# microsoft/VidTok

Measured on NVIDIA H100. Metric: frames/sec encode+decode, kl_causal_488 17x256x256, higher is better.
Workload: dtype bf16

## Files before the change

### vidtok_b200/csrc/tblock_tc.cu

```cuda
#include <cuda.h>

#include <cstdio>
#include <cstdlib>
#include <cstring>
#include <string>

#include "common.cuh"
#include "kernels.h"
#include "tc_ptx.cuh"

namespace vt {

namespace {
using namespace tcx;

thread_local std::string g_tb_err;
constexpr int kC = 128;
constexpr int kKc = kC / 64;
constexpr uint32_t kTile = 128 * 128;
constexpr int kHSlots = 3;
constexpr int kConsumerWarps = 8;
constexpr int kProducerWarp = kConsumerWarps;
constexpr int kThreadsTb = (kConsumerWarps + 4) * 32;

struct TbParams {
  int B, T, H, W;
  int BW, BH;
  int tilesW, tilesH;
  long long num_strips;
  int stages;
  const float* bias1;
  const float* bias2;
  const float* g2;
  const float* b2;
  int ln_out, ln_out_silu;
  const float* g3;
  const float* b3;
  const bf16* x;
  bf16* out;
  bf16* out2;
  const bf16* n1;
  int cached_in;
  const bf16* cn1_in;
  const bf16* ch_in;
  bf16* cn1_out;
  bf16* ch_out;
};
struct TbMaps {
  CUtensorMap n1, w1, w2, cn1;
};

__device__ __forceinline__ float quad_sum(float v) {
  v += __shfl_xor_sync(0xffffffffu, v, 1);
  v += __shfl_xor_sync(0xffffffffu, v, 2);
  return v;
}

template <bool kCache>
__global__ void __launch_bounds__(kThreadsTb, 1) tblock_tc_kernel(const __grid_constant__ TbMaps maps, const TbParams p) {
  extern __shared__ uint8_t smem_raw[];
  const uint32_t smem_base = (smem_u32(smem_raw) + 1023u) & ~1023u;
  uint8_t* smem_gen = smem_raw + (smem_base - smem_u32(smem_raw));
  const int warp = threadIdx.x >> 5, lane = threadIdx.x & 31;
  const uint32_t h_base = smem_base;
  const uint32_t ring_base = h_base + kHSlots * kKc * kTile;
  const uint32_t stage_bytes = 2u * kTile;
  const uint32_t bar_base = ring_base + (uint32_t)p.stages * stage_bytes;
  auto full_bar = [&](int s) { return bar_base + 8u * s; };
  auto empty_bar = [&](int s) { return bar_base + 8u * (p.stages + s); };
  float* cst = reinterpret_cast<float*>(smem_gen + (bar_base - smem_base) + 16u * p.stages);

  for (int i = threadIdx.x; i < kC; i += kThreadsTb) {
    cst[i] = p.bias1 ? p.bias1[i] : 0.f;
    cst[kC + i] = 0.5f * p.g2[i];
    cst[2 * kC + i] = 0.5f * p.b2[i];
    cst[3 * kC + i] = p.bias2 ? p.bias2[i] : 0.f;
    const float sc = p.ln_out_silu ? 0.5f : 1.0f;
    cst[4 * kC + i] = p.ln_out ? sc * p.g3[i] : 0.f;
    cst[5 * kC + i] = p.ln_out ? sc * p.b3[i] : 0.f;
  }
  if (threadIdx.x == 0) {
    for (int s = 0; s < p.stages; ++s) { mbar_init(full_bar(s), 1); mbar_init(empty_bar(s), kConsumerWarps); }
    asm volatile("fence.mbarrier_init.release.cluster;" ::: "memory");
  }
  __syncthreads();

  if (warp >= kProducerWarp) {
    asm volatile("setmaxnreg.dec.sync.aligned.u32 40;" ::: "memory");
    if (warp != kProducerWarp) return;
    const bool el = elect_one();
    if (el) { prefetch_tmap(&maps.n1); prefetch_tmap(&maps.w1); prefetch_tmap(&maps.w2); }
    const bool front = kCache && p.cached_in;
    int stage = 0;
    uint32_t phase = 0;
    auto acquire = [&](uint32_t bytes) {
      mbar_wait(empty_bar(stage), phase ^ 1u);
      if (el) mbar_expect_tx(full_bar(stage), bytes);
    };
    auto advance = [&]() { if (++stage == p.stages) { stage = 0; phase ^= 1u; } };
    for (long long strip = blockIdx.x; strip < p.num_strips; strip += gridDim.x) {
      const int tw = (int)(strip % p.tilesW);
      const int th = (int)((strip / p.tilesW) % p.tilesH);
      const int b = (int)(strip / ((long long)p.tilesW * p.tilesH));
      const int w0 = tw * p.BW, h0 = th * p.BH;
      for (int t = 0; t < p.T; ++t) {
        for (int a = 0; a < 3; ++a) {
          const int tv = t - 2 + a;
          if (tv < 0 && !front) continue;
          for (int kc = 0; kc < kKc; ++kc) {
            acquire(2u * kTile);
            if (el) {
              const uint32_t sa = ring_base + stage * stage_bytes;
              if (kCache && tv < 0) tma_load_5d(sa, &maps.cn1, full_bar(stage), kc * 64, w0, h0, tv + 2, b);
              else tma_load_5d(sa, &maps.n1, full_bar(stage), kc * 64, w0, h0, tv, b);
              tma_load_3d(sa + kTile, &maps.w1, full_bar(stage), a * kC + kc * 64, 0, 0);
            }
            advance();
          }
        }
        for (int a = 0; a < 3; ++a) {
          if (t - 2 + a < 0 && !front) continue;
          for (int kc = 0; kc < kKc; ++kc) {
            acquire(kTile);
            if (el) tma_load_3d(ring_base + stage * stage_bytes + kTile, &maps.w2, full_bar(stage), a * kC + kc * 64, 0, 0);
            advance();
          }
        }
      }
    }
    return;
  }

  asm volatile("setmaxnreg.inc.sync.aligned.u32 232;" ::: "memory");
  const int g = warp >> 2, wq = warp & 3;
  const uint32_t hi = desc_hi(1024u);
  float acc[kC / 2];
  int stage = 0, pend_stage = -1;
  uint32_t phase = 0;
  auto release = [&]() {
    if (lane == 0 && pend_stage >= 0) mbar_arrive(empty_bar(pend_stage));
    pend_stage = -1;
  };
  auto kstep = [&](bool a_from_stage, uint32_t h_addr, uint32_t scale) {
    mbar_wait(full_bar(stage), phase);
    const uint32_t sa = ring_base + stage * stage_bytes;
    const uint32_t al = desc_lo(a_from_stage ? sa + (uint32_t)g * 64u * 128u : h_addr), bl = desc_lo(sa + kTile);
    wgmma_fence();
#pragma unroll
    for (uint32_t j = 0; j < 4u; ++j) wgmma_k16<kC, false>(acc, desc(al + 2u * j, hi), desc(bl + 2u * j, hi), j == 0 ? scale : 1u);
    wgmma_commit();
    wgmma_wait<1>();
    release();
    pend_stage = stage;
    if (++stage == p.stages) { stage = 0; phase ^= 1u; }
  };
  auto finish = [&]() {
    wgmma_wait<0>();
    acc_fence(acc);
    release();
  };
  auto wg_sync = [&]() { asm volatile("bar.sync %0, 128;" ::"r"(1 + g) : "memory"); };
  const float* bias1 = cst;
  const float* g2 = cst + kC;
  const float* b2 = cst + 2 * kC;
  const float* bias2 = cst + 3 * kC;
  const float* g3 = cst + 4 * kC;
  const float* b3 = cst + 5 * kC;
  const int cq = 2 * (lane & 3);
  const int rbase = 64 * g + 16 * wq + (lane >> 2);
  const bool front = kCache && p.cached_in;
  const int gtid = threadIdx.x & 127;
  auto slot_of = [&](int tv) { return h_base + (uint32_t)((tv + kHSlots) % kHSlots) * kKc * kTile; };
  auto ring_unit = [&](uint32_t slot, int row, int c) {
    return reinterpret_cast<uint4*>(smem_gen + (slot - smem_base) + (c >> 6) * kTile + row * 128 + ((((c & 63) >> 3) ^ (row & 7)) << 4));
  };

  for (long long strip = blockIdx.x; strip < p.num_strips; strip += gridDim.x) {
    const int tw = (int)(strip % p.tilesW);
    const int th = (int)((strip / p.tilesW) % p.tilesH);
    const int b = (int)(strip / ((long long)p.tilesW * p.tilesH));
    long long pos0[2];
#pragma unroll
    for (int r = 0; r < 2; ++r) {
      const int row = rbase + 8 * r;
      const int h = th * p.BH + row / p.BW, w = tw * p.BW + row % p.BW;
      pos0[r] = (((long long)b * p.T) * p.H + h) * p.W + w;
    }
    const long long frame = (long long)p.H * p.W;
    auto cache_pos = [&](int i, int j, int& row) {
      row = 64 * g + (i >> 4);
      const int h = th * p.BH + row / p.BW, w = tw * p.BW + row % p.BW;
      return ((((long long)b * 2 + j) * p.H + h) * p.W + w) * kC + (i & 15) * 8;
    };
    if (front) {
      wg_sync();
      for (int j = 0; j < 2; ++j)
        for (int i = gtid; i < 64 * 16; i += 128) {
          int row;
          const long long off = cache_pos(i, j, row);
          *ring_unit(slot_of(j - 2), row, (i & 15) * 8) = *reinterpret_cast<const uint4*>(p.ch_in + off);
        }
      fence_async_smem();
      wg_sync();
    }
    for (int t = 0; t < p.T; ++t) {
      uint32_t scale = 0;
      for (int a = 0; a < 3; ++a) {
        if (t - 2 + a < 0 && !front) continue;
        for (int kc = 0; kc < kKc; ++kc) { kstep(true, 0u, scale); scale = 1; }
      }
      finish();
      wg_sync();
      const uint32_t slot = h_base + (uint32_t)(t % kHSlots) * kKc * kTile;
#pragma unroll
      for (int r = 0; r < 2; ++r) {
        float s = 0.f, q = 0.f;
#pragma unroll
        for (int j = 0; j < kC / 8; ++j) {
          const int c = 8 * j + cq;
          const float f0 = acc[4 * j + 2 * r] + bias1[c], f1 = acc[4 * j + 2 * r + 1] + bias1[c + 1];
          s += f0 + f1;
          q = fmaf(f0, f0, q);
          q = fmaf(f1, f1, q);
          const uint32_t kp = pack_bf16x2(f0, f1);
          acc[4 * j + 2 * r] = bf16_lo(kp);
          acc[4 * j + 2 * r + 1] = bf16_hi(kp);
        }
        const float mean = quad_sum(s) * (1.0f / kC);
        float var = fmaf(-mean, mean, quad_sum(q) * (1.0f / kC));
        var = var < 0.f ? 0.f : var;
        const float rstd = rsqrtf(var + 1e-6f);
        const float nmr = -mean * rstd;
        const int row = rbase + 8 * r;
        uint8_t* hrow = smem_gen + (slot - smem_base) + row * 128;
#pragma unroll
        for (int j = 0; j < kC / 8; ++j) {
          const int c = 8 * j + cq;
          float y0 = fmaf(fmaf(acc[4 * j + 2 * r], rstd, nmr), g2[c], b2[c]);
          float y1 = fmaf(fmaf(acc[4 * j + 2 * r + 1], rstd, nmr), g2[c + 1], b2[c + 1]);
          y0 = fmaf(y0, tanh_approx(y0), y0);
          y1 = fmaf(y1, tanh_approx(y1), y1);
          const int cc = c & 63, u = cc >> 3;
          *reinterpret_cast<uint32_t*>(hrow + (c >> 6) * kTile + ((u ^ (row & 7)) << 4) + (cc & 7) * 2) = pack_bf16x2(y0, y1);
        }
      }
      fence_async_smem();
      wg_sync();
      scale = 0;
      for (int a = 0; a < 3; ++a) {
        const int tv = t - 2 + a;
        if (tv < 0 && !front) continue;
        const uint32_t hs = (kCache ? slot_of(tv) : h_base + (uint32_t)(tv % kHSlots) * kKc * kTile) + (uint32_t)g * 64u * 128u;
        for (int kc = 0; kc < kKc; ++kc) { kstep(false, hs + (uint32_t)kc * kTile, scale); scale = 1; }
      }
      finish();
#pragma unroll
      for (int r = 0; r < 2; ++r) {
        const long long off = (pos0[r] + (long long)t * frame) * kC;
        const bf16* xr = p.x + off;
        bf16* orow = p.out + off;
        float s = 0.f, q = 0.f;
#pragma unroll
        for (int j = 0; j < kC / 8; ++j) {
          const int c = 8 * j + cq;
          const uint32_t xw = *reinterpret_cast<const uint32_t*>(xr + c);
          const float f0 = acc[4 * j + 2 * r] + bias2[c] + bf16_lo(xw), f1 = acc[4 * j + 2 * r + 1] + bias2[c + 1] + bf16_hi(xw);
          s += f0 + f1;
          q = fmaf(f0, f0, q);
          q = fmaf(f1, f1, q);
          const uint32_t kp = pack_bf16x2(f0, f1);
          *reinterpret_cast<uint32_t*>(orow + c) = kp;
          acc[4 * j + 2 * r] = bf16_lo(kp);
          acc[4 * j + 2 * r + 1] = bf16_hi(kp);
        }
        if (!p.ln_out) continue;
        const float mean = quad_sum(s) * (1.0f / kC);
        float var = fmaf(-mean, mean, quad_sum(q) * (1.0f / kC));
        var = var < 0.f ? 0.f : var;
        const float rstd = rsqrtf(var + 1e-6f);
        const float nmr = -mean * rstd;
        bf16* o2 = p.out2 + off;
#pragma unroll
        for (int j = 0; j < kC / 8; ++j) {
          const int c = 8 * j + cq;
          float y0 = fmaf(fmaf(acc[4 * j + 2 * r], rstd, nmr), g3[c], b3[c]);
          float y1 = fmaf(fmaf(acc[4 * j + 2 * r + 1], rstd, nmr), g3[c + 1], b3[c + 1]);
          if (p.ln_out_silu) {
            y0 = fmaf(y0, tanh_approx(y0), y0);
            y1 = fmaf(y1, tanh_approx(y1), y1);
          }
          *reinterpret_cast<uint32_t*>(o2 + c) = pack_bf16x2(y0, y1);
        }
      }
    }
    if (kCache) {
      for (int j = 0; j < 2; ++j) {
        const int tv = p.T - 2 + j;
        for (int i = gtid; i < 64 * 16; i += 128) {
          int row;
          const long long off = cache_pos(i, j, row);
          const long long pix = off - (((long long)b * 2 + j) * frame) * kC;
          uint4 hv = make_uint4(0u, 0u, 0u, 0u), nv = hv;
          if (tv >= 0 || front) hv = *ring_unit(slot_of(tv), row, (i & 15) * 8);
          if (tv >= 0) nv = *reinterpret_cast<const uint4*>(p.n1 + (((long long)b * p.T + tv) * frame) * kC + pix);
          else if (front) nv = *reinterpret_cast<const uint4*>(p.cn1_in + (((long long)b * 2 + tv + 2) * frame) * kC + pix);
          *reinterpret_cast<uint4*>(p.ch_out + off) = hv;
          *reinterpret_cast<uint4*>(p.cn1_out + off) = nv;
        }
      }
    }
  }
}

typedef CUresult (*EncodeTiledFn)(CUtensorMap*, CUtensorMapDataType, cuuint32_t, void*, const cuuint64_t*,
                                  const cuuint64_t*, const cuuint32_t*, const cuuint32_t*, CUtensorMapInterleave,
                                  CUtensorMapSwizzle, CUtensorMapL2promotion, CUtensorMapFloatOOBfill);
EncodeTiledFn tb_get_encode() {
  static EncodeTiledFn fn = nullptr;
  static bool tried = false;
  if (!tried) {
    tried = true;
    void* f = nullptr;
    cudaDriverEntryPointQueryResult q;
    if (cudaGetDriverEntryPoint("cuTensorMapEncodeTiled", &f, cudaEnableDefault, &q) == cudaSuccess && q == cudaDriverEntryPointSuccess)
      fn = (EncodeTiledFn)f;
  }
  return fn;
}

bool strip_box(int H, int W, int& BW, int& BH) {
  for (int bw = 128; bw >= 1; bw >>= 1) {
    if (W % bw != 0) continue;
    const int bh = 128 / bw;
    if (bh <= 256 && H % bh == 0) { BW = bw; BH = bh; return true; }
  }
  return false;
}
}

const char* tblock_tc_last_error() { return g_tb_err.c_str(); }

bool tblock_tc_supported(int B, int T, int H, int W, int C, bool planning) {
// ... 3 lines not shown
  if (!env) { g_tb_err = "disabled (VT_TBLOCK=0)"; return false; }
  if (C != kC) { g_tb_err = "C != 128"; return false; }
  if (B <= 0 || T <= 0) { g_tb_err = "empty"; return false; }
  int BW, BH;
  if (!strip_box(H, W, BW, BH)) { g_tb_err = "H x W not tileable by a 128-position box"; return false; }
  if (!planning && !tb_get_encode()) { g_tb_err = "cuTensorMapEncodeTiled unavailable"; return false; }
  return true;
}

cudaError_t launch_tblock_tc(const bf16* n1, const bf16* x, const bf16* w1, const float* bias1, const float* gamma2,
                             const float* beta2, const bf16* w2, const float* bias2, bf16* out, bf16* out2,
                             const float* gamma_out, const float* beta_out, bool out_silu, int B, int T, int H, int W,
                             cudaStream_t s, const TbCache* cache) {
  g_tb_err.clear();
  EncodeTiledFn enc = tb_get_encode();
  if (!enc) { g_tb_err = "cuTensorMapEncodeTiled unavailable"; return cudaErrorNotSupported; }
  TbParams p;
  memset(&p, 0, sizeof(p));
  if (!strip_box(H, W, p.BW, p.BH)) { g_tb_err = "H x W not tileable"; return cudaErrorInvalidValue; }
  p.B = B; p.T = T; p.H = H; p.W = W;
  p.tilesW = W / p.BW; p.tilesH = H / p.BH;
  p.num_strips = (long long)B * p.tilesH * p.tilesW;
  p.bias1 = bias1; p.bias2 = bias2; p.g2 = gamma2; p.b2 = beta2;
  p.ln_out = (out2 && gamma_out && beta_out) ? 1 : 0;
  p.ln_out_silu = out_silu ? 1 : 0;
  p.g3 = gamma_out; p.b3 = beta_out;
  p.x = x; p.out = out; p.out2 = out2;
  if (cache) {
    if (!cache->n1_out || !cache->h_out || (!cache->n1_in != !cache->h_in)) { g_tb_err = "cache: both outputs, and both or no inputs"; return cudaErrorInvalidValue; }
    p.n1 = n1;
    p.cached_in = cache->n1_in ? 1 : 0;
    p.cn1_in = cache->n1_in; p.ch_in = cache->h_in; p.cn1_out = cache->n1_out; p.ch_out = cache->h_out;
  }
  const size_t fixed = 1024 + (size_t)kHSlots * kKc * kTile + 6 * kC * 4;
  const size_t budget = 225 * 1024;
  int stages = (int)((budget - fixed) / (2 * kTile + 16));
  if (stages > 4) stages = 4;
  p.stages = stages;
  const size_t smem = fixed + (size_t)stages * (2 * kTile + 16);
  TbMaps maps;
  {
    cuuint64_t dims[5] = {(cuuint64_t)kC, (cuuint64_t)W, (cuuint64_t)H, (cuuint64_t)T, (cuuint64_t)B};
    cuuint64_t strides[4] = {(cuuint64_t)kC * 2, (cuuint64_t)W * kC * 2, (cuuint64_t)H * W * kC * 2, (cuuint64_t)T * H * W * kC * 2};
    cuuint32_t box[5] = {64, (cuuint32_t)p.BW, (cuuint32_t)p.BH, 1, 1};
    cuuint32_t es[5] = {1, 1, 1, 1, 1};
    CUresult r = enc(&maps.n1, CU_TENSOR_MAP_DATA_TYPE_BFLOAT16, 5, const_cast<bf16*>(n1), dims, strides, box, es, CU_TENSOR_MAP_INTERLEAVE_NONE,
                     CU_TENSOR_MAP_SWIZZLE_128B, CU_TENSOR_MAP_L2_PROMOTION_L2_256B, CU_TENSOR_MAP_FLOAT_OOB_FILL_NONE);
    if (r != CUDA_SUCCESS) { g_tb_err = "cuTensorMapEncodeTiled(n1) failed: " + std::to_string((int)r); return cudaErrorInvalidValue; }
    maps.cn1 = maps.n1;
    if (p.cached_in) {
      dims[3] = 2;
      strides[3] = 2ull * H * W * kC * 2;
      r = enc(&maps.cn1, CU_TENSOR_MAP_DATA_TYPE_BFLOAT16, 5, const_cast<bf16*>(p.cn1_in), dims, strides, box, es, CU_TENSOR_MAP_INTERLEAVE_NONE,
              CU_TENSOR_MAP_SWIZZLE_128B, CU_TENSOR_MAP_L2_PROMOTION_L2_256B, CU_TENSOR_MAP_FLOAT_OOB_FILL_NONE);
      if (r != CUDA_SUCCESS) { g_tb_err = "cuTensorMapEncodeTiled(n1 cache) failed: " + std::to_string((int)r); return cudaErrorInvalidValue; }
    }
  }
  for (int i = 0; i < 2; ++i) {
    cuuint64_t dims[3] = {(cuuint64_t)(3 * kC), (cuuint64_t)kC, 1};
    cuuint64_t strides[2] = {(cuuint64_t)(3 * kC) * 2, (cuuint64_t)(3 * kC) * kC * 2};
    cuuint32_t box[3] = {64, (cuuint32_t)kC, 1};
    cuuint32_t es[3] = {1, 1, 1};
    CUresult r = enc(i ? &maps.w2 : &maps.w1, CU_TENSOR_MAP_DATA_TYPE_BFLOAT16, 3, const_cast<bf16*>(i ? w2 : w1), dims, strides, box, es,
                     CU_TENSOR_MAP_INTERLEAVE_NONE, CU_TENSOR_MAP_SWIZZLE_128B, CU_TENSOR_MAP_L2_PROMOTION_L2_256B,
                     CU_TENSOR_MAP_FLOAT_OOB_FILL_NONE);
    if (r != CUDA_SUCCESS) { g_tb_err = "cuTensorMapEncodeTiled(weights) failed: " + std::to_string((int)r); return cudaErrorInvalidValue; }
  }
  static bool attr[64] = {false};
  static int sms[64] = {0};
  int dev = 0;
  cudaGetDevice(&dev);
  if (dev < 0 || dev >= 64) return cudaErrorInvalidDevice;
// ... 23 lines not shown
```

Before: 435.9.

## Process two frames per step so each weight tile feeds two WGMMA accumulators

Restructures the fused temporal block kernel to handle frame pairs. Each weight tile loaded through TMA is now reused for two output frames with two accumulator sets. The ring becomes single-tile slots (weights and activations loaded separately), and the h ring grows to four slots so both frames' history fits. The aim is to halve weight-tile traffic and barrier round trips per frame. Epilogue constants move from shared memory to __ldg reads, and an L2 prefetch of the residual input is added. The cost is doubled accumulator registers, which raises spill risk under the 232-register cap, and fewer effective pipeline stages.

```diff
diff --git a/vidtok_b200/csrc/tblock_tc.cu b/vidtok_b200/csrc/tblock_tc.cu
--- a/vidtok_b200/csrc/tblock_tc.cu
+++ b/vidtok_b200/csrc/tblock_tc.cu
@@ -4,6 +4,7 @@
 #include <cstdlib>
 #include <cstring>
 #include <string>
+#include <type_traits>
 
 #include "common.cuh"
 #include "kernels.h"
@@ -18,7 +19,8 @@
 constexpr int kC = 128;
 constexpr int kKc = kC / 64;
 constexpr uint32_t kTile = 128 * 128;
-constexpr int kHSlots = 3;
+constexpr int kHSlots = 4;
+constexpr int kTiles = 6;
 constexpr int kConsumerWarps = 8;
 constexpr int kProducerWarp = kConsumerWarps;
 constexpr int kThreadsTb = (kConsumerWarps + 4) * 32;
@@ -28,7 +30,6 @@
   int BW, BH;
   int tilesW, tilesH;
   long long num_strips;
-  int stages;
   const float* bias1;
   const float* bias2;
   const float* g2;
@@ -55,6 +56,12 @@
   v += __shfl_xor_sync(0xffffffffu, v, 2);
   return v;
 }
+template <typename T>
+__device__ __forceinline__ const T* opaque(const T* p) {
+  asm volatile("" : "+l"(p));
+  return p;
+}
+__device__ __forceinline__ void prefetch_l2(const void* p) { asm volatile("prefetch.global.L2 [%0];" ::"l"(p)); }
 
 template <bool kCache>
 __global__ void __launch_bounds__(kThreadsTb, 1) tblock_tc_kernel(const __grid_constant__ TbMaps maps, const TbParams p) {
@@ -64,68 +71,64 @@
   const int warp = threadIdx.x >> 5, lane = threadIdx.x & 31;
   const uint32_t h_base = smem_base;
   const uint32_t ring_base = h_base + kHSlots * kKc * kTile;
-  const uint32_t stage_bytes = 2u * kTile;
-  const uint32_t bar_base = ring_base + (uint32_t)p.stages * stage_bytes;
+  const uint32_t bar_base = ring_base + kTiles * kTile;
   auto full_bar = [&](int s) { return bar_base + 8u * s; };
-  auto empty_bar = [&](int s) { return bar_base + 8u * (p.stages + s); };
-  float* cst = reinterpret_cast<float*>(smem_gen + (bar_base - smem_base) + 16u * p.stages);
-
-  for (int i = threadIdx.x; i < kC; i += kThreadsTb) {
-    cst[i] = p.bias1 ? p.bias1[i] : 0.f;
-    cst[kC + i] = 0.5f * p.g2[i];
-    cst[2 * kC + i] = 0.5f * p.b2[i];
-    cst[3 * kC + i] = p.bias2 ? p.bias2[i] : 0.f;
-    const float sc = p.ln_out_silu ? 0.5f : 1.0f;
-    cst[4 * kC + i] = p.ln_out ? sc * p.g3[i] : 0.f;
-    cst[5 * kC + i] = p.ln_out ? sc * p.b3[i] : 0.f;
-  }
+  auto empty_bar = [&](int s) { return bar_base + 8u * (kTiles + s); };
   if (threadIdx.x == 0) {
-    for (int s = 0; s < p.stages; ++s) { mbar_init(full_bar(s), 1); mbar_init(empty_bar(s), kConsumerWarps); }
+    for (int s = 0; s < kTiles; ++s) { mbar_init(full_bar(s), 1); mbar_init(empty_bar(s), kConsumerWarps); }
     asm volatile("fence.mbarrier_init.release.cluster;" ::: "memory");
   }
   __syncthreads();
+  const bool front = kCache && p.cached_in;
 
   if (warp >= kProducerWarp) {
     asm volatile("setmaxnreg.dec.sync.aligned.u32 40;" ::: "memory");
     if (warp != kProducerWarp) return;
     const bool el = elect_one();
     if (el) { prefetch_tmap(&maps.n1); prefetch_tmap(&maps.w1); prefetch_tmap(&maps.w2); }
-    const bool front = kCache && p.cached_in;
-    int stage = 0;
+    int tile = 0;
     uint32_t phase = 0;
-    auto acquire = [&](uint32_t bytes) {
-      mbar_wait(empty_bar(stage), phase ^ 1u);
-      if (el) mbar_expect_tx(full_bar(stage), bytes);
+    auto acquire = [&]() {
+      mbar_wait(empty_bar(tile), phase ^ 1u);
+      if (el) mbar_expect_tx(full_bar(tile), kTile);
+      return ring_base + (uint32_t)tile * kTile;
     };
-    auto advance = [&]() { if (++stage == p.stages) { stage = 0; phase ^= 1u; } };
+    auto advance = [&]() { if (++tile == kTiles) { tile = 0; phase ^= 1u; } };
     for (long long strip = blockIdx.x; strip < p.num_strips; strip += gridDim.x) {
       const int tw = (int)(strip % p.tilesW);
       const int th = (int)((strip / p.tilesW) % p.tilesH);
       const int b = (int)(strip / ((long long)p.tilesW * p.tilesH));
       const int w0 = tw * p.BW, h0 = th * p.BH;
-      for (int t = 0; t < p.T; ++t) {
+      for (int t0 = 0; t0 < p.T; t0 += 2) {
+        const int nf = p.T - t0 < 2 ? 1 : 2;
         for (int a = 0; a < 3; ++a) {
-          const int tv = t - 2 + a;
-          if (tv < 0 && !front) continue;
+          const bool v0 = t0 - 2 + a >= 0 || front, v1 = nf > 1 && (t0 - 1 + a >= 0 || front);
+          if (!v0 && !v1) continue;
           for (int kc = 0; kc < kKc; ++kc) {
-            acquire(2u * kTile);
-            if (el) {
-              const uint32_t sa = ring_base + stage * stage_bytes;
-              if (kCache && tv < 0) tma_load_5d(sa, &maps.cn1, full_bar(stage), kc * 64, w0, h0, tv + 2, b);
-              else tma_load_5d(sa, &maps.n1, full_bar(stage), kc * 64, w0, h0, tv, b);
-              tma_load_3d(sa + kTile, &maps.w1, full_bar(stage), a * kC + kc * 64, 0, 0);
+            uint32_t sa = acquire();
+            if (el) tma_load_3d(sa, &maps.w1, full_bar(tile), a * kC + kc * 64, 0, 0);
+            advance();
+            for (int f = 0; f < 2; ++f) {
+              if (!(f ? v1 : v0)) continue;
+              const int tv = t0 + f - 2 + a;
+              sa = acquire();
+              if (el) {
+                if (kCache && tv < 0) tma_load_5d(sa, &maps.cn1, full_bar(tile), kc * 64, w0, h0, tv + 2, b);
+                else tma_load_5d(sa, &maps.n1, full_bar(tile), kc * 64, w0, h0, tv, b);
+              }
+              advance();
             }
+          }
+        }
+        for (int a = 0; a < 3; ++a) {
+          const bool v0 = t0 - 2 + a >= 0 || front, v1 = nf > 1 && (t0 - 1 + a >= 0 || front);
+          if (!v0 && !v1) continue;
+          for (int kc = 0; kc < kKc; ++kc) {
+            const uint32_t sa = acquire();
+            if (el) tma_load_3d(sa, &maps.w2, full_bar(tile), a * kC + kc * 64, 0, 0);
             advance();
           }
         }
-        for (int a = 0; a < 3; ++a) {
-          if (t - 2 + a < 0 && !front) continue;
-          for (int kc = 0; kc < kKc; ++kc) {
-            acquire(kTile);
-            if (el) tma_load_3d(ring_base + stage * stage_bytes + kTile, &maps.w2, full_bar(stage), a * kC + kc * 64, 0, 0);
-            advance();
-          }
-        }
       }
     }
     return;
@@ -134,45 +137,153 @@
   asm volatile("setmaxnreg.inc.sync.aligned.u32 232;" ::: "memory");
   const int g = warp >> 2, wq = warp & 3;
   const uint32_t hi = desc_hi(1024u);
-  float acc[kC / 2];
-  int stage = 0, pend_stage = -1;
+  float acc[2][kC / 2];
+  int tile = 0, pend_first = 0, pend_n = 0;
   uint32_t phase = 0;
+  auto take = [&]() {
+    mbar_wait(full_bar(tile), phase);
+    const uint32_t a = ring_base + (uint32_t)tile * kTile;
+    if (++tile == kTiles) { tile = 0; phase ^= 1u; }
+    return a;
+  };
   auto release = [&]() {
-    if (lane == 0 && pend_stage >= 0) mbar_arrive(empty_bar(pend_stage));
-    pend_stage = -1;
-  };
-  auto kstep = [&](bool a_from_stage, uint32_t h_addr, uint32_t scale) {
-    mbar_wait(full_bar(stage), phase);
-    const uint32_t sa = ring_base + stage * stage_bytes;
-    const uint32_t al = desc_lo(a_from_stage ? sa + (uint32_t)g * 64u * 128u : h_addr), bl = desc_lo(sa + kTile);
+    int tt = pend_first;
+    for (int i = 0; i < pend_n; ++i) {
+      if (lane == 0) mbar_arrive(empty_bar(tt));
+      tt = tt + 1 == kTiles ? 0 : tt + 1;
+    }
+    pend_n = 0;
+  };
+  uint32_t scale0 = 0, scale1 = 0;
+  auto kstep_impl = [&](auto v0c, auto v1c, bool g1, uint32_t h0, uint32_t h1) {
+    constexpr bool V0 = decltype(v0c)::value, V1 = decltype(v1c)::value;
+    const int first = tile;
+    const uint32_t bl = desc_lo(take());
+    uint32_t a0 = h0, a1 = h1;
+    if (g1) {
+      if (V0) a0 = take() + (uint32_t)g * 64u * 128u;
+      if (V1) a1 = take() + (uint32_t)g * 64u * 128u;
+    }
+    const uint32_t al0 = desc_lo(a0), al1 = desc_lo(a1);
     wgmma_fence();
 #pragma unroll
-    for (uint32_t j = 0; j < 4u; ++j) wgmma_k16<kC, false>(acc, desc(al + 2u * j, hi), desc(bl + 2u * j, hi), j == 0 ? scale : 1u);
+    for (uint32_t j = 0; j < 4u; ++j) {
+      if (V0) wgmma_k16<kC, false>(acc[0], desc(al0 + 2u * j, hi), desc(bl + 2u * j, hi), j == 0 ? scale0 : 1u);
+      if (V1) wgmma_k16<kC, false>(acc[1], desc(al1 + 2u * j, hi), desc(bl + 2u * j, hi), j == 0 ? scale1 : 1u);
+    }
     wgmma_commit();
+    if (V0) scale0 = 1;
+    if (V1) scale1 = 1;
     wgmma_wait<1>();
     release();
-    pend_stage = stage;
-    if (++stage == p.stages) { stage = 0; phase ^= 1u; }
+    pend_first = first;
+    pend_n = 1 + (g1 ? (int)V0 + (int)V1 : 0);
+  };
+  using T1 = std::true_type;
+  using F1 = std::false_type;
+  auto kstep = [&](bool g1, bool v0, bool v1, uint32_t h0, uint32_t h1) {
+    if (v0 && v1) kstep_impl(T1{}, T1{}, g1, h0, h1);
+    else if (v1) kstep_impl(F1{}, T1{}, g1, h0, h1);
+    else kstep_impl(T1{}, F1{}, g1, h0, h1);
   };
   auto finish = [&]() {
     wgmma_wait<0>();
-    acc_fence(acc);
+    acc_fence(acc[0]);
+    acc_fence(acc[1]);
     release();
   };
   auto wg_sync = [&]() { asm volatile("bar.sync %0, 128;" ::"r"(1 + g) : "memory"); };
-  const float* bias1 = cst;
-  const float* g2 = cst + kC;
-  const float* b2 = cst + 2 * kC;
-  const float* bias2 = cst + 3 * kC;
-  const float* g3 = cst + 4 * kC;
-  const float* b3 = cst + 5 * kC;
   const int cq = 2 * (lane & 3);
   const int rbase = 64 * g + 16 * wq + (lane >> 2);
-  const bool front = kCache && p.cached_in;
   const int gtid = threadIdx.x & 127;
   auto slot_of = [&](int tv) { return h_base + (uint32_t)((tv + kHSlots) % kHSlots) * kKc * kTile; };
   auto ring_unit = [&](uint32_t slot, int row, int c) {
     return reinterpret_cast<uint4*>(smem_gen + (slot - smem_base) + (c >> 6) * kTile + row * 128 + ((((c & 63) >> 3) ^ (row & 7)) << 4));
+  };
+  const long long frame = (long long)p.H * p.W;
+
+  auto e1 = [&](float (&ac)[kC / 2], int tv) {
+    const uint32_t slot = slot_of(tv);
+    const float* bias1 = p.bias1 ? opaque(p.bias1) + cq : nullptr;
+    const float* g2 = opaque(p.g2) + cq;
+    const float* b2 = opaque(p.b2) + cq;
+#pragma unroll
+    for (int r = 0; r < 2; ++r) {
+      float s = 0.f, q = 0.f;
+#pragma unroll
+      for (int j = 0; j < kC / 8; ++j) {
+        const float f0 = ac[4 * j + 2 * r] + (bias1 ? __ldg(bias1 + 8 * j) : 0.f);
+        const float f1 = ac[4 * j + 2 * r + 1] + (bias1 ? __ldg(bias1 + 8 * j + 1) : 0.f);
+        s += f0 + f1;
+        q = fmaf(f0, f0, q);
+        q = fmaf(f1, f1, q);
+        const uint32_t kp = pack_bf16x2(f0, f1);
+        ac[4 * j + 2 * r] = bf16_lo(kp);
+        ac[4 * j + 2 * r + 1] = bf16_hi(kp);
+      }
+      const float mean = quad_sum(s) * (1.0f / kC);
+      float var = fmaf(-mean, mean, quad_sum(q) * (1.0f / kC));
+      var = var < 0.f ? 0.f : var;
+      const float rstd = rsqrtf(var + 1e-6f);
+      const float nmr = -mean * rstd;
+      const int row = rbase + 8 * r;
+      uint8_t* hrow = smem_gen + (slot - smem_base) + row * 128;
+#pragma unroll
+      for (int j = 0; j < kC / 8; ++j) {
+        const int c = 8 * j + cq;
+        float y0 = fmaf(fmaf(ac[4 * j + 2 * r], rstd, nmr), 0.5f * __ldg(g2 + 8 * j), 0.5f * __ldg(b2 + 8 * j));
+        float y1 = fmaf(fmaf(ac[4 * j + 2 * r + 1], rstd, nmr), 0.5f * __ldg(g2 + 8 * j + 1), 0.5f * __ldg(b2 + 8 * j + 1));
+        y0 = fmaf(y0, tanh_approx(y0), y0);
+        y1 = fmaf(y1, tanh_approx(y1), y1);
+        const int cc = c & 63, u = cc >> 3;
+        *reinterpret_cast<uint32_t*>(hrow + (c >> 6) * kTile + ((u ^ (row & 7)) << 4) + (cc & 7) * 2) = pack_bf16x2(y0, y1);
+      }
+    }
+  };
+  auto e2 = [&](float (&ac)[kC / 2], const long long (&pos)[2], int t) {
+    const float* bias2 = p.bias2 ? opaque(p.bias2) + cq : nullptr;
+    const float* g3 = p.ln_out ? opaque(p.g3) + cq : nullptr;
+    const float* b3 = p.ln_out ? opaque(p.b3) + cq : nullptr;
+    const float sc = p.ln_out_silu ? 0.5f : 1.0f;
+#pragma unroll
+    for (int r = 0; r < 2; ++r) {
+      const long long off = (pos[r] + (long long)t * frame) * kC;
+      const bf16* xr = p.x + off;
+      bf16* orow = p.out + off;
+      float s = 0.f, q = 0.f;
+#pragma unroll
+      for (int j = 0; j < kC / 8; ++j) {
+        const int c = 8 * j + cq;
+        const uint32_t xw = *reinterpret_cast<const uint32_t*>(xr + c);
+        const float f0 = ac[4 * j + 2 * r] + (bias2 ? __ldg(bias2 + 8 * j) : 0.f) + bf16_lo(xw);
+        const float f1 = ac[4 * j + 2 * r + 1] + (bias2 ? __ldg(bias2 + 8 * j + 1) : 0.f) + bf16_hi(xw);
+        s += f0 + f1;
+        q = fmaf(f0, f0, q);
+        q = fmaf(f1, f1, q);
+        const uint32_t kp = pack_bf16x2(f0, f1);
+        *reinterpret_cast<uint32_t*>(orow + c) = kp;
+        ac[4 * j + 2 * r] = bf16_lo(kp);
+        ac[4 * j + 2 * r + 1] = bf16_hi(kp);
+      }
+      if (!p.ln_out) continue;
+      const float mean = quad_sum(s) * (1.0f / kC);
+      float var = fmaf(-mean, mean, quad_sum(q) * (1.0f / kC));
+      var = var < 0.f ? 0.f : var;
+      const float rstd = rsqrtf(var + 1e-6f);
+      const float nmr = -mean * rstd;
+      bf16* o2 = p.out2 + off;
+#pragma unroll
+      for (int j = 0; j < kC / 8; ++j) {
+        const int c = 8 * j + cq;
+        float y0 = fmaf(fmaf(ac[4 * j + 2 * r], rstd, nmr), sc * __ldg(g3 + 8 * j), sc * __ldg(b3 + 8 * j));
+        float y1 = fmaf(fmaf(ac[4 * j + 2 * r + 1], rstd, nmr), sc * __ldg(g3 + 8 * j + 1), sc * __ldg(b3 + 8 * j + 1));
+        if (p.ln_out_silu) {
+          y0 = fmaf(y0, tanh_approx(y0), y0);
+          y1 = fmaf(y1, tanh_approx(y1), y1);
+        }
+        *reinterpret_cast<uint32_t*>(o2 + c) = pack_bf16x2(y0, y1);
+      }
+    }
   };
 
   for (long long strip = blockIdx.x; strip < p.num_strips; strip += gridDim.x) {
@@ -186,7 +297,6 @@
       const int h = th * p.BH + row / p.BW, w = tw * p.BW + row % p.BW;
       pos0[r] = (((long long)b * p.T) * p.H + h) * p.W + w;
     }
-    const long long frame = (long long)p.H * p.W;
     auto cache_pos = [&](int i, int j, int& row) {
       row = 64 * g + (i >> 4);
       const int h = th * p.BH + row / p.BW, w = tw * p.BW + row % p.BW;
@@ -203,95 +313,32 @@
       fence_async_smem();
       wg_sync();
     }
-    for (int t = 0; t < p.T; ++t) {
-      uint32_t scale = 0;
+    for (int t0 = 0; t0 < p.T; t0 += 2) {
+      const int nf = p.T - t0 < 2 ? 1 : 2;
+      scale0 = scale1 = 0;
       for (int a = 0; a < 3; ++a) {
-        if (t - 2 + a < 0 && !front) continue;
-        for (int kc = 0; kc < kKc; ++kc) { kstep(true, 0u, scale); scale = 1; }
+        const bool v0 = t0 - 2 + a >= 0 || front, v1 = nf > 1 && (t0 - 1 + a >= 0 || front);
+        if (!v0 && !v1) continue;
+        for (int kc = 0; kc < kKc; ++kc) kstep(true, v0, v1, 0u, 0u);
       }
       finish();
       wg_sync();
-      const uint32_t slot = h_base + (uint32_t)(t % kHSlots) * kKc * kTile;
-#pragma unroll
-      for (int r = 0; r < 2; ++r) {
-        float s = 0.f, q = 0.f;
-#pragma unroll
-        for (int j = 0; j < kC / 8; ++j) {
-          const int c = 8 * j + cq;
-          const float f0 = acc[4 * j + 2 * r] + bias1[c], f1 = acc[4 * j + 2 * r + 1] + bias1[c + 1];
-          s += f0 + f1;
-          q = fmaf(f0, f0, q);
-          q = fmaf(f1, f1, q);
-          const uint32_t kp = pack_bf16x2(f0, f1);
-          acc[4 * j + 2 * r] = bf16_lo(kp);
-          acc[4 * j + 2 * r + 1] = bf16_hi(kp);
-        }
-        const float mean = quad_sum(s) * (1.0f / kC);
-        float var = fmaf(-mean, mean, quad_sum(q) * (1.0f / kC));
-        var = var < 0.f ? 0.f : var;
-        const float rstd = rsqrtf(var + 1e-6f);
-        const float nmr = -mean * rstd;
-        const int row = rbase + 8 * r;
-        uint8_t* hrow = smem_gen + (slot - smem_base) + row * 128;
-#pragma unroll
-        for (int j = 0; j < kC / 8; ++j) {
-          const int c = 8 * j + cq;
-          float y0 = fmaf(fmaf(acc[4 * j + 2 * r], rstd, nmr), g2[c], b2[c]);
-          float y1 = fmaf(fmaf(acc[4 * j + 2 * r + 1], rstd, nmr), g2[c + 1], b2[c + 1]);
-          y0 = fmaf(y0, tanh_approx(y0), y0);
-          y1 = fmaf(y1, tanh_approx(y1), y1);
-          const int cc = c & 63, u = cc >> 3;
-          *reinterpret_cast<uint32_t*>(hrow + (c >> 6) * kTile + ((u ^ (row & 7)) << 4) + (cc & 7) * 2) = pack_bf16x2(y0, y1);
-        }
-      }
+      e1(acc[0], t0);
+      if (nf > 1) e1(acc[1], t0 + 1);
       fence_async_smem();
       wg_sync();
-      scale = 0;
+      for (int f = 0; f < nf; ++f)
+        prefetch_l2(p.x + (((lane >> 1) & 1 ? pos0[1] : pos0[0]) + (long long)(t0 + f) * frame) * kC + 64 * (lane & 1));
+      scale0 = scale1 = 0;
       for (int a = 0; a < 3; ++a) {
-        const int tv = t - 2 + a;
-        if (tv < 0 && !front) continue;
-        const uint32_t hs = (kCache ? slot_of(tv) : h_base + (uint32_t)(tv % kHSlots) * kKc * kTile) + (uint32_t)g * 64u * 128u;
-        for (int kc = 0; kc < kKc; ++kc) { kstep(false, hs + (uint32_t)kc * kTile, scale); scale = 1; }
+        const bool v0 = t0 - 2 + a >= 0 || front, v1 = nf > 1 && (t0 - 1 + a >= 0 || front);
+        if (!v0 && !v1) continue;
+        const uint32_t hs0 = slot_of(t0 - 2 + a) + (uint32_t)g * 64u * 128u, hs1 = slot_of(t0 - 1 + a) + (uint32_t)g * 64u * 128u;
+        for (int kc = 0; kc < kKc; ++kc) kstep(false, v0, v1, hs0 + (uint32_t)kc * kTile, hs1 + (uint32_t)kc * kTile);
       }
       finish();
-#pragma unroll
-      for (int r = 0; r < 2; ++r) {
-        const long long off = (pos0[r] + (long long)t * frame) * kC;
-        const bf16* xr = p.x + off;
-        bf16* orow = p.out + off;
-        float s = 0.f, q = 0.f;
-#pragma unroll
-        for (int j = 0; j < kC / 8; ++j) {
-          const int c = 8 * j + cq;
-          const uint32_t xw = *reinterpret_cast<const uint32_t*>(xr + c);
-          const float f0 = acc[4 * j + 2 * r] + bias2[c] + bf16_lo(xw), f1 = acc[4 * j + 2 * r + 1] + bias2[c + 1] + bf16_hi(xw);
-          s += f0 + f1;
-          q = fmaf(f0, f0, q);
-          q = fmaf(f1, f1, q);
-          const uint32_t kp = pack_bf16x2(f0, f1);
-          *reinterpret_cast<uint32_t*>(orow + c) = kp;
-          acc[4 * j + 2 * r] = bf16_lo(kp);
-          acc[4 * j + 2 * r + 1] = bf16_hi(kp);
-        }
-        if (!p.ln_out) continue;
-        const float mean = quad_sum(s) * (1.0f / kC);
-        float var = fmaf(-mean, mean, quad_sum(q) * (1.0f / kC));
-        var = var < 0.f ? 0.f : var;
-        const float rstd = rsqrtf(var + 1e-6f);
-        const float nmr = -mean * rstd;
-        bf16* o2 = p.out2 + off;
-#pragma unroll
-        for (int j = 0; j < kC / 8; ++j) {
-          const int c = 8 * j + cq;
-          float y0 = fmaf(fmaf(acc[4 * j + 2 * r], rstd, nmr), g3[c], b3[c]);
-          float y1 = fmaf(fmaf(acc[4 * j + 2 * r + 1], rstd, nmr), g3[c + 1], b3[c + 1]);
-          if (p.ln_out_silu) {
-            y0 = fmaf(y0, tanh_approx(y0), y0);
-            y1 = fmaf(y1, tanh_approx(y1), y1);
-          }
-          *reinterpret_cast<uint32_t*>(o2 + c) = pack_bf16x2(y0, y1);
-        }
-      }
+      e2(acc[0], pos0, t0);
+      if (nf > 1) e2(acc[1], pos0, t0 + 1);
     }
     if (kCache) {
       for (int j = 0; j < 2; ++j) {
@@ -377,12 +424,8 @@
     p.cached_in = cache->n1_in ? 1 : 0;
     p.cn1_in = cache->n1_in; p.ch_in = cache->h_in; p.cn1_out = cache->n1_out; p.ch_out = cache->h_out;
   }
-  const size_t fixed = 1024 + (size_t)kHSlots * kKc * kTile + 6 * kC * 4;
-  const size_t budget = 225 * 1024;
-  int stages = (int)((budget - fixed) / (2 * kTile + 16));
-  if (stages > 4) stages = 4;
-  p.stages = stages;
-  const size_t smem = fixed + (size_t)stages * (2 * kTile + 16);
+  const size_t smem = 1024 + (size_t)kHSlots * kKc * kTile + (size_t)kTiles * kTile + 16 * kTiles;
+  static_assert(1024 + (size_t)kHSlots * kKc * kTile + (size_t)kTiles * kTile + 16 * kTiles <= 227 * 1024, "tblock_tc smem plan");
   TbMaps maps;
   {
     cuuint64_t dims[5] = {(cuuint64_t)kC, (cuuint64_t)W, (cuuint64_t)H, (cuuint64_t)T, (cuuint64_t)B};
```

Result: no change. 435.7 (median of 6 runs) (-0.1%).

## Ping-pong two consumer warpgroups over time steps with single-tile operand ring

Applied to the files above, without the earlier changes.

Restructures the temporal block kernel so each consumer warpgroup owns whole time-step items (128 rows, two accumulators) and the two warpgroups alternate GEMM turns via named barriers. The epilogue of one group can then overlap with the tensor-core work of the other. The ring now holds single tiles (A and B as separate entries), the ring grows to up to 8 entries, and the h history grows to 4 slots. It also prefetches the residual x to L2 and batches its loads before the epilogue. Register pressure doubles for accumulators, and the barrier/skip phase bookkeeping is intricate, with risk of deadlock or ordering bugs.

```diff
diff --git a/vidtok_b200/csrc/tblock_tc.cu b/vidtok_b200/csrc/tblock_tc.cu
--- a/vidtok_b200/csrc/tblock_tc.cu
+++ b/vidtok_b200/csrc/tblock_tc.cu
@@ -18,17 +18,19 @@
 constexpr int kC = 128;
 constexpr int kKc = kC / 64;
 constexpr uint32_t kTile = 128 * 128;
-constexpr int kHSlots = 3;
+constexpr int kHSlots = 4;
+constexpr int kMaxEntries = 8;
 constexpr int kConsumerWarps = 8;
 constexpr int kProducerWarp = kConsumerWarps;
 constexpr int kThreadsTb = (kConsumerWarps + 4) * 32;
+constexpr uint32_t kBarTurn = 1, kBarWg = 3, kBarDrain = 5;
 
 struct TbParams {
   int B, T, H, W;
   int BW, BH;
   int tilesW, tilesH;
   long long num_strips;
-  int stages;
+  int entries;
   const float* bias1;
   const float* bias2;
   const float* g2;
@@ -64,11 +66,11 @@
   const int warp = threadIdx.x >> 5, lane = threadIdx.x & 31;
   const uint32_t h_base = smem_base;
   const uint32_t ring_base = h_base + kHSlots * kKc * kTile;
-  const uint32_t stage_bytes = 2u * kTile;
-  const uint32_t bar_base = ring_base + (uint32_t)p.stages * stage_bytes;
+  const int E = p.entries;
+  const uint32_t bar_base = ring_base + (uint32_t)E * kTile;
   auto full_bar = [&](int s) { return bar_base + 8u * s; };
-  auto empty_bar = [&](int s) { return bar_base + 8u * (p.stages + s); };
-  float* cst = reinterpret_cast<float*>(smem_gen + (bar_base - smem_base) + 16u * p.stages);
+  auto empty_bar = [&](int s) { return bar_base + 8u * (E + s); };
+  float* cst = reinterpret_cast<float*>(smem_gen + (bar_base - smem_base) + 16u * E);
 
   for (int i = threadIdx.x; i < kC; i += kThreadsTb) {
     cst[i] = p.bias1 ? p.bias1[i] : 0.f;
@@ -80,53 +82,68 @@
     cst[5 * kC + i] = p.ln_out ? sc * p.b3[i] : 0.f;
   }
   if (threadIdx.x == 0) {
-    for (int s = 0; s < p.stages; ++s) { mbar_init(full_bar(s), 1); mbar_init(empty_bar(s), kConsumerWarps); }
+    for (int s = 0; s < E; ++s) { mbar_init(full_bar(s), 1); mbar_init(empty_bar(s), kConsumerWarps / 2); }
     asm volatile("fence.mbarrier_init.release.cluster;" ::: "memory");
   }
   __syncthreads();
+
+  const bool front = kCache && p.cached_in;
+  const long long n_items = (p.num_strips - blockIdx.x + gridDim.x - 1) / gridDim.x * p.T;
+  auto taps = [&](int t) { return front ? 3 : (t < 2 ? t + 1 : 3); };
 
   if (warp >= kProducerWarp) {
     asm volatile("setmaxnreg.dec.sync.aligned.u32 40;" ::: "memory");
     if (warp != kProducerWarp) return;
     const bool el = elect_one();
-    if (el) { prefetch_tmap(&maps.n1); prefetch_tmap(&maps.w1); prefetch_tmap(&maps.w2); }
-    const bool front = kCache && p.cached_in;
+    if (el) { prefetch_tmap(&maps.n1); prefetch_tmap(&maps.w1); prefetch_tmap(&maps.w2); if (front) prefetch_tmap(&maps.cn1); }
     int stage = 0;
     uint32_t phase = 0;
-    auto acquire = [&](uint32_t bytes) {
+    auto acquire = [&]() {
       mbar_wait(empty_bar(stage), phase ^ 1u);
-      if (el) mbar_expect_tx(full_bar(stage), bytes);
+      if (el) mbar_expect_tx(full_bar(stage), kTile);
     };
-    auto advance = [&]() { if (++stage == p.stages) { stage = 0; phase ^= 1u; } };
-    for (long long strip = blockIdx.x; strip < p.num_strips; strip += gridDim.x) {
+    auto advance = [&]() { if (++stage == E) { stage = 0; phase ^= 1u; } };
+    auto load_g1 = [&](long long i) {
+      const long long strip = blockIdx.x + (i / p.T) * gridDim.x;
+      const int t = (int)(i % p.T);
       const int tw = (int)(strip % p.tilesW);
       const int th = (int)((strip / p.tilesW) % p.tilesH);
       const int b = (int)(strip / ((long long)p.tilesW * p.tilesH));
       const int w0 = tw * p.BW, h0 = th * p.BH;
-      for (int t = 0; t < p.T; ++t) {
-        for (int a = 0; a < 3; ++a) {
-          const int tv = t - 2 + a;
-          if (tv < 0 && !front) continue;
-          for (int kc = 0; kc < kKc; ++kc) {
-            acquire(2u * kTile);
-            if (el) {
-              const uint32_t sa = ring_base + stage * stage_bytes;
-              if (kCache && tv < 0) tma_load_5d(sa, &maps.cn1, full_bar(stage), kc * 64, w0, h0, tv + 2, b);
-              else tma_load_5d(sa, &maps.n1, full_bar(stage), kc * 64, w0, h0, tv, b);
-              tma_load_3d(sa + kTile, &maps.w1, full_bar(stage), a * kC + kc * 64, 0, 0);
-            }
-            advance();
+      for (int a = 0; a < 3; ++a) {
+        const int tv = t - 2 + a;
+        if (tv < 0 && !front) continue;
+        for (int kc = 0; kc < kKc; ++kc) {
+          acquire();
+          if (el) {
+            const uint32_t sa = ring_base + stage * kTile;
+            if (kCache && tv < 0) tma_load_5d(sa, &maps.cn1, full_bar(stage), kc * 64, w0, h0, tv + 2, b);
+            else tma_load_5d(sa, &maps.n1, full_bar(stage), kc * 64, w0, h0, tv, b);
           }
-        }
-        for (int a = 0; a < 3; ++a) {
-          if (t - 2 + a < 0 && !front) continue;
-          for (int kc = 0; kc < kKc; ++kc) {
-            acquire(kTile);
-            if (el) tma_load_3d(ring_base + stage * stage_bytes + kTile, &maps.w2, full_bar(stage), a * kC + kc * 64, 0, 0);
-            advance();
-          }
+          advance();
+          acquire();
+          if (el) tma_load_3d(ring_base + stage * kTile, &maps.w1, full_bar(stage), a * kC + kc * 64, 0, 0);
+          advance();
         }
       }
+    };
+    auto load_g2 = [&](long long i) {
+      const int t = (int)(i % p.T);
+      for (int a = 0; a < 3; ++a) {
+        if (t - 2 + a < 0 && !front) continue;
+        for (int kc = 0; kc < kKc; ++kc) {
+          acquire();
+          if (el) tma_load_3d(ring_base + stage * kTile, &maps.w2, full_bar(stage), a * kC + kc * 64, 0, 0);
+          advance();
+        }
+      }
+    };
+    for (long long i = 0; i < n_items; i += 2) {
+      const bool pair = i + 1 < n_items;
+      load_g1(i);
+      if (pair) load_g1(i + 1);
+      load_g2(i);
+      if (pair) load_g2(i + 1);
     }
     return;
   }
@@ -134,32 +151,53 @@
   asm volatile("setmaxnreg.inc.sync.aligned.u32 232;" ::: "memory");
   const int g = warp >> 2, wq = warp & 3;
   const uint32_t hi = desc_hi(1024u);
-  float acc[kC / 2];
-  int stage = 0, pend_stage = -1;
+  float acc[2][kC / 2];
+  int stage = 0, pend_stage = -1, pend_n = 0;
   uint32_t phase = 0;
   auto release = [&]() {
-    if (lane == 0 && pend_stage >= 0) mbar_arrive(empty_bar(pend_stage));
+    if (lane == 0 && pend_stage >= 0) {
+      mbar_arrive(empty_bar(pend_stage));
+      if (pend_n == 2) mbar_arrive(empty_bar(pend_stage + 1 == E ? 0 : pend_stage + 1));
+    }
     pend_stage = -1;
   };
-  auto kstep = [&](bool a_from_stage, uint32_t h_addr, uint32_t scale) {
+  auto next_entry = [&]() { if (++stage == E) { stage = 0; phase ^= 1u; } };
+  auto skip = [&](int n) {
+    stage += n;
+    if ((stage / E) & 1) phase ^= 1u;
+    stage %= E;
+  };
+  auto kstep = [&](bool a_from_ring, uint32_t h_addr, uint32_t scale) {
+    const int s0 = stage;
+    uint32_t a_addr = h_addr;
+    if (a_from_ring) {
+      mbar_wait(full_bar(stage), phase);
+      a_addr = ring_base + stage * kTile;
+      next_entry();
+    }
     mbar_wait(full_bar(stage), phase);
-    const uint32_t sa = ring_base + stage * stage_bytes;
-    const uint32_t al = desc_lo(a_from_stage ? sa + (uint32_t)g * 64u * 128u : h_addr), bl = desc_lo(sa + kTile);
+    const uint32_t al = desc_lo(a_addr), bl = desc_lo(ring_base + stage * kTile);
+    next_entry();
     wgmma_fence();
 #pragma unroll
-    for (uint32_t j = 0; j < 4u; ++j) wgmma_k16<kC, false>(acc, desc(al + 2u * j, hi), desc(bl + 2u * j, hi), j == 0 ? scale : 1u);
+    for (uint32_t j = 0; j < 4u; ++j) {
+      const uint64_t bh = desc(bl + 2u * j, hi);
+      wgmma_k16<kC, false>(acc[0], desc(al + 2u * j, hi), bh, j == 0 ? scale : 1u);
+      wgmma_k16<kC, false>(acc[1], desc(al + ((64u * 128u) >> 4) + 2u * j, hi), bh, j == 0 ? scale : 1u);
+    }
     wgmma_commit();
     wgmma_wait<1>();
     release();
-    pend_stage = stage;
-    if (++stage == p.stages) { stage = 0; phase ^= 1u; }
+    pend_stage = s0;
+    pend_n = a_from_ring ? 2 : 1;
   };
   auto finish = [&]() {
     wgmma_wait<0>();
-    acc_fence(acc);
+    acc_fence(acc[0]);
+    acc_fence(acc[1]);
     release();
   };
-  auto wg_sync = [&]() { asm volatile("bar.sync %0, 128;" ::"r"(1 + g) : "memory"); };
+  auto wg_sync = [&]() { named_bar_sync(kBarWg + g, 128); };
   const float* bias1 = cst;
   const float* g2 = cst + kC;
   const float* b2 = cst + 2 * kC;
@@ -167,111 +205,137 @@
   const float* g3 = cst + 4 * kC;
   const float* b3 = cst + 5 * kC;
   const int cq = 2 * (lane & 3);
-  const int rbase = 64 * g + 16 * wq + (lane >> 2);
-  const bool front = kCache && p.cached_in;
+  const int rbase = 16 * wq + (lane >> 2);
   const int gtid = threadIdx.x & 127;
-  auto slot_of = [&](int tv) { return h_base + (uint32_t)((tv + kHSlots) % kHSlots) * kKc * kTile; };
+  const long long frame = (long long)p.H * p.W;
   auto ring_unit = [&](uint32_t slot, int row, int c) {
     return reinterpret_cast<uint4*>(smem_gen + (slot - smem_base) + (c >> 6) * kTile + row * 128 + ((((c & 63) >> 3) ^ (row & 7)) << 4));
   };
 
-  for (long long strip = blockIdx.x; strip < p.num_strips; strip += gridDim.x) {
+  for (long long i = g; i < n_items; i += 2) {
+    const bool has_next = i + 1 < n_items;
+    const long long k = i / p.T;
+    const int t = (int)(i % p.T);
+    const long long strip = blockIdx.x + k * gridDim.x;
     const int tw = (int)(strip % p.tilesW);
     const int th = (int)((strip / p.tilesW) % p.tilesH);
     const int b = (int)(strip / ((long long)p.tilesW * p.tilesH));
-    long long pos0[2];
-#pragma unroll
-    for (int r = 0; r < 2; ++r) {
-      const int row = rbase + 8 * r;
+    const long long hv = kCache ? k * (p.T + 2) + 2 : k * p.T;
+    auto slot_of = [&](int tv) { return h_base + ((uint32_t)(hv + tv) & (kHSlots - 1)) * kKc * kTile; };
+    auto cache_pos = [&](int u, int j, int& row) {
+      row = u >> 4;
       const int h = th * p.BH + row / p.BW, w = tw * p.BW + row % p.BW;
-      pos0[r] = (((long long)b * p.T) * p.H + h) * p.W + w;
-    }
-    const long long frame = (long long)p.H * p.W;
-    auto cache_pos = [&](int i, int j, int& row) {
-      row = 64 * g + (i >> 4);
+      return ((((long long)b * 2 + j) * p.H + h) * p.W + w) * kC + (u & 15) * 8;
+    };
+    auto pos_off = [&](int row) {
       const int h = th * p.BH + row / p.BW, w = tw * p.BW + row % p.BW;
-      return ((((long long)b * 2 + j) * p.H + h) * p.W + w) * kC + (i & 15) * 8;
+      return ((((long long)b * p.T + t) * p.H + h) * p.W + w) * kC;
     };
-    if (front) {
-      wg_sync();
+#pragma unroll
+    for (int l = 0; l < 2; ++l) {
+      const int line = gtid + 128 * l;
+      asm volatile("prefetch.global.L2 [%0];" ::"l"(p.x + pos_off(line >> 1) + (line & 1) * 64));
+    }
+
+    if (g == 1) skip(2 * kKc * taps(t == 0 ? p.T - 1 : t - 1));
+    if (i > 0) named_bar_sync(kBarTurn + g, kConsumerWarps * 32);
+    uint32_t scale = 0;
+    for (int a = 0; a < 3; ++a) {
+      if (t - 2 + a < 0 && !front) continue;
+      for (int kc = 0; kc < kKc; ++kc) { kstep(true, 0u, scale); scale = 1; }
+    }
+    if (g == 1 || has_next) named_bar_arrive(kBarTurn + (g ^ 1), kConsumerWarps * 32);
+    finish();
+    if (kCache && t == 0 && i > 0) named_bar_sync(kBarDrain + (g ^ 1), kConsumerWarps * 32);
+    wg_sync();
+    if (front && t == 0) {
       for (int j = 0; j < 2; ++j)
-        for (int i = gtid; i < 64 * 16; i += 128) {
+        for (int u = gtid; u < 128 * 16; u += 128) {
           int row;
-          const long long off = cache_pos(i, j, row);
-          *ring_unit(slot_of(j - 2), row, (i & 15) * 8) = *reinterpret_cast<const uint4*>(p.ch_in + off);
-        }
-      fence_async_smem();
-      wg_sync();
-    }
-    for (int t = 0; t < p.T; ++t) {
-      uint32_t scale = 0;
-      for (int a = 0; a < 3; ++a) {
-        if (t - 2 + a < 0 && !front) continue;
-        for (int kc = 0; kc < kKc; ++kc) { kstep(true, 0u, scale); scale = 1; }
-      }
-      finish();
-      wg_sync();
-      const uint32_t slot = h_base + (uint32_t)(t % kHSlots) * kKc * kTile;
+          const long long off = cache_pos(u, j, row);
+          *ring_unit(slot_of(j - 2), row, (u & 15) * 8) = *reinterpret_cast<const uint4*>(p.ch_in + off);
+        }
+    }
+    const uint32_t slot = slot_of(t);
+#pragma unroll
+    for (int hf = 0; hf < 2; ++hf) {
+      float (&ah)[kC / 2] = acc[hf];
 #pragma unroll
       for (int r = 0; r < 2; ++r) {
         float s = 0.f, q = 0.f;
 #pragma unroll
         for (int j = 0; j < kC / 8; ++j) {
           const int c = 8 * j + cq;
-          const float f0 = acc[4 * j + 2 * r] + bias1[c], f1 = acc[4 * j + 2 * r + 1] + bias1[c + 1];
+          const float f0 = ah[4 * j + 2 * r] + bias1[c], f1 = ah[4 * j + 2 * r + 1] + bias1[c + 1];
           s += f0 + f1;
           q = fmaf(f0, f0, q);
           q = fmaf(f1, f1, q);
           const uint32_t kp = pack_bf16x2(f0, f1);
-          acc[4 * j + 2 * r] = bf16_lo(kp);
-          acc[4 * j + 2 * r + 1] = bf16_hi(kp);
+          ah[4 * j + 2 * r] = bf16_lo(kp);
+          ah[4 * j + 2 * r + 1] = bf16_hi(kp);
         }
         const float mean = quad_sum(s) * (1.0f / kC);
         float var = fmaf(-mean, mean, quad_sum(q) * (1.0f / kC));
         var = var < 0.f ? 0.f : var;
         const float rstd = rsqrtf(var + 1e-6f);
         const float nmr = -mean * rstd;
-        const int row = rbase + 8 * r;
+        const int row = rbase + 64 * hf + 8 * r;
         uint8_t* hrow = smem_gen + (slot - smem_base) + row * 128;
 #pragma unroll
         for (int j = 0; j < kC / 8; ++j) {
           const int c = 8 * j + cq;
-          float y0 = fmaf(fmaf(acc[4 * j + 2 * r], rstd, nmr), g2[c], b2[c]);
-          float y1 = fmaf(fmaf(acc[4 * j + 2 * r + 1], rstd, nmr), g2[c + 1], b2[c + 1]);
+          float y0 = fmaf(fmaf(ah[4 * j + 2 * r], rstd, nmr), g2[c], b2[c]);
+          float y1 = fmaf(fmaf(ah[4 * j + 2 * r + 1], rstd, nmr), g2[c + 1], b2[c + 1]);
           y0 = fmaf(y0, tanh_approx(y0), y0);
           y1 = fmaf(y1, tanh_approx(y1), y1);
           const int cc = c & 63, u = cc >> 3;
           *reinterpret_cast<uint32_t*>(hrow + (c >> 6) * kTile + ((u ^ (row & 7)) << 4) + (cc & 7) * 2) = pack_bf16x2(y0, y1);
         }
       }
-      fence_async_smem();
-      wg_sync();
-      scale = 0;
-      for (int a = 0; a < 3; ++a) {
-        const int tv = t - 2 + a;
-        if (tv < 0 && !front) continue;
-        const uint32_t hs = (kCache ? slot_of(tv) : h_base + (uint32_t)(tv % kHSlots) * kKc * kTile) + (uint32_t)g * 64u * 128u;
-        for (int kc = 0; kc < kKc; ++kc) { kstep(false, hs + (uint32_t)kc * kTile, scale); scale = 1; }
+    }
+    fence_async_smem();
+    wg_sync();
+    if (g == 0) { if (has_next) skip(2 * kKc * taps(t + 1 == p.T ? 0 : t + 1)); }
+    else skip(kKc * taps(t == 0 ? p.T - 1 : t - 1));
+    if (g == 1 || has_next) named_bar_sync(kBarTurn + g, kConsumerWarps * 32);
+    scale = 0;
+    for (int a = 0; a < 3; ++a) {
+      const int tv = t - 2 + a;
+      if (tv < 0 && !front) continue;
+      const uint32_t hs = slot_of(tv);
+      for (int kc = 0; kc < kKc; ++kc) { kstep(false, hs + (uint32_t)kc * kTile, scale); scale = 1; }
+    }
+    if (has_next) named_bar_arrive(kBarTurn + (g ^ 1), kConsumerWarps * 32);
+    finish();
+    if (g == 0 && has_next) skip(kKc * taps(t + 1 == p.T ? 0 : t + 1));
+#pragma unroll
+    for (int hf = 0; hf < 2; ++hf) {
+      float (&ah)[kC / 2] = acc[hf];
+      int row0 = rbase + 64 * hf;
+      asm volatile("" : "+r"(row0));
+      uint32_t xw[2][kC / 8];
+#pragma unroll
+      for (int r = 0; r < 2; ++r) {
+        const uint32_t* xr = reinterpret_cast<const uint32_t*>(p.x + pos_off(row0 + 8 * r) + cq);
+#pragma unroll
+        for (int j = 0; j < kC / 8; ++j) xw[r][j] = __ldg(xr + 4 * j);
       }
-      finish();
 #pragma unroll
       for (int r = 0; r < 2; ++r) {
-        const long long off = (pos0[r] + (long long)t * frame) * kC;
-        const bf16* xr = p.x + off;
+        const long long off = pos_off(row0 + 8 * r);
         bf16* orow = p.out + off;
         float s = 0.f, q = 0.f;
 #pragma unroll
         for (int j = 0; j < kC / 8; ++j) {
           const int c = 8 * j + cq;
-          const uint32_t xw = *reinterpret_cast<const uint32_t*>(xr + c);
-          const float f0 = acc[4 * j + 2 * r] + bias2[c] + bf16_lo(xw), f1 = acc[4 * j + 2 * r + 1] + bias2[c + 1] + bf16_hi(xw);
+          const float f0 = ah[4 * j + 2 * r] + bias2[c] + bf16_lo(xw[r][j]), f1 = ah[4 * j + 2 * r + 1] + bias2[c + 1] + bf16_hi(xw[r][j]);
           s += f0 + f1;
           q = fmaf(f0, f0, q);
           q = fmaf(f1, f1, q);
           const uint32_t kp = pack_bf16x2(f0, f1);
           *reinterpret_cast<uint32_t*>(orow + c) = kp;
-          acc[4 * j + 2 * r] = bf16_lo(kp);
-          acc[4 * j + 2 * r + 1] = bf16_hi(kp);
+          ah[4 * j + 2 * r] = bf16_lo(kp);
+          ah[4 * j + 2 * r + 1] = bf16_hi(kp);
         }
         if (!p.ln_out) continue;
         const float mean = quad_sum(s) * (1.0f / kC);
@@ -283,8 +347,8 @@
 #pragma unroll
         for (int j = 0; j < kC / 8; ++j) {
           const int c = 8 * j + cq;
-          float y0 = fmaf(fmaf(acc[4 * j + 2 * r], rstd, nmr), g3[c], b3[c]);
-          float y1 = fmaf(fmaf(acc[4 * j + 2 * r + 1], rstd, nmr), g3[c + 1], b3[c + 1]);
+          float y0 = fmaf(fmaf(ah[4 * j + 2 * r], rstd, nmr), g3[c], b3[c]);
+          float y1 = fmaf(fmaf(ah[4 * j + 2 * r + 1], rstd, nmr), g3[c + 1], b3[c + 1]);
           if (p.ln_out_silu) {
             y0 = fmaf(y0, tanh_approx(y0), y0);
             y1 = fmaf(y1, tanh_approx(y1), y1);
@@ -293,21 +357,22 @@
         }
       }
     }
-    if (kCache) {
+    if (kCache && t == p.T - 1) {
       for (int j = 0; j < 2; ++j) {
         const int tv = p.T - 2 + j;
-        for (int i = gtid; i < 64 * 16; i += 128) {
+        for (int u = gtid; u < 128 * 16; u += 128) {
           int row;
-          const long long off = cache_pos(i, j, row);
+          const long long off = cache_pos(u, j, row);
           const long long pix = off - (((long long)b * 2 + j) * frame) * kC;
-          uint4 hv = make_uint4(0u, 0u, 0u, 0u), nv = hv;
-          if (tv >= 0 || front) hv = *ring_unit(slot_of(tv), row, (i & 15) * 8);
+          uint4 hv4 = make_uint4(0u, 0u, 0u, 0u), nv = hv4;
+          if (tv >= 0 || front) hv4 = *ring_unit(slot_of(tv), row, (u & 15) * 8);
           if (tv >= 0) nv = *reinterpret_cast<const uint4*>(p.n1 + (((long long)b * p.T + tv) * frame) * kC + pix);
           else if (front) nv = *reinterpret_cast<const uint4*>(p.cn1_in + (((long long)b * 2 + tv + 2) * frame) * kC + pix);
-          *reinterpret_cast<uint4*>(p.ch_out + off) = hv;
+          *reinterpret_cast<uint4*>(p.ch_out + off) = hv4;
           *reinterpret_cast<uint4*>(p.cn1_out + off) = nv;
         }
       }
+      if (has_next) named_bar_arrive(kBarDrain + g, kConsumerWarps * 32);
     }
   }
 }
@@ -378,11 +443,12 @@
     p.cn1_in = cache->n1_in; p.ch_in = cache->h_in; p.cn1_out = cache->n1_out; p.ch_out = cache->h_out;
   }
   const size_t fixed = 1024 + (size_t)kHSlots * kKc * kTile + 6 * kC * 4;
-  const size_t budget = 225 * 1024;
-  int stages = (int)((budget - fixed) / (2 * kTile + 16));
-  if (stages > 4) stages = 4;
-  p.stages = stages;
-  const size_t smem = fixed + (size_t)stages * (2 * kTile + 16);
+  const size_t budget = 227 * 1024;
+  int entries = (int)((budget - fixed) / (kTile + 16));
+  if (entries > kMaxEntries) entries = kMaxEntries;
+  if (entries < 4) { g_tb_err = "shared memory too small for the operand ring"; return cudaErrorInvalidValue; }
+  p.entries = entries;
+  const size_t smem = fixed + (size_t)entries * (kTile + 16);
   TbMaps maps;
   {
     cuuint64_t dims[5] = {(cuuint64_t)kC, (cuuint64_t)W, (cuuint64_t)H, (cuuint64_t)T, (cuuint64_t)B};
```

Result: faster. 330.4 before, 337.8 after (median of 6 runs) (+2.3%).
